# CompVis/unsupervised-part-segmentation

Measured on AMD Instinct MI355X. Metric: images/sec training (CUB 128x128, 10 parts), higher is better.
Workload: dtype bf16

## Files before the change

include/upsparts_hip.h:

```cpp
#ifndef UPSPARTS_HIP_H
#define UPSPARTS_HIP_H

#include <stddef.h>
#include <stdint.h>

#ifdef __cplusplus
extern "C" {
#endif

#define UPS_ABI_VERSION 6

enum { UPS_F32 = 0, UPS_BF16 = 1, UPS_F16 = 2 };
enum { UPS_ACT_NONE = 0, UPS_ACT_LRELU = 1, UPS_ACT_RELU = 2, UPS_ACT_ELU = 3 };
enum { UPS_OK = 0, UPS_E_ARG = -1, UPS_E_UNSUPPORTED = -2, UPS_E_LAUNCH = -3 };

int ups_abi_version(void);
void ups_struct_sizes(int64_t out[4]);
const char* ups_last_error(void);

typedef struct {
    int32_t dtype;
    int32_t n, hi, wi;
    int32_t ci;
    int32_t ldi;
// ... 137 lines not shown
int ups_act_mean_fwd(const void* x, void* y, int32_t dtype, int32_t n, int32_t hw, int32_t c, int32_t act, float slope, void* stream);
int ups_act_mean_bwd(const void* x, const void* gy, void* gx, int32_t dtype, int32_t n, int32_t hw, int32_t c, int32_t act, float slope, void* stream);
int ups_maxpool2_fwd(const void* x, void* y, int32_t dtype, int32_t n, int32_t h, int32_t w, int32_t c, void* stream);
int ups_maxpool2_fwd_f8(const void* x, void* y, int32_t n, int32_t h, int32_t w, int32_t c, void* y_f8, const float* scale,
                        float* amax, int32_t act, float slope, void* stream);
int ups_maxpool2_bwd(const void* x, const void* gy, void* gx, int32_t dtype, int32_t n, int32_t h, int32_t w, int32_t c, void* stream);
int ups_copy_channels(const void* src, int32_t lds, void* dst, int32_t ldd, int32_t dtype, int64_t rows, int32_t c, void* stream);
int ups_add_channels(const void* src, int32_t lds, void* dst, int32_t ldd, int32_t dtype, int64_t rows, int32_t c, void* stream);

int ups_vgg_preprocess_fwd(const void* x, int32_t x_is_f32, int32_t ldx, void* y, int32_t dtype, int64_t pixels, void* stream);
int ups_vgg_preprocess_bwd(const void* gy, void* gx, int32_t dtype, int32_t ldgx, int64_t pixels, void* stream);
int ups_l1_fwd(const void* a, const void* b, int32_t dtype, int64_t rows, int32_t c, int32_t ld, int32_t act,
               float* partial, int32_t nblocks, void* stream);
int ups_l1_bwd(const void* a, const void* b, void* gb, int32_t dtype, int64_t rows, int32_t c, int32_t ld, int32_t act,
               const float* scale_dev, float scale, void* stream);
int ups_sum_scale(const float* partial, int32_t n, float scale, float* out, int32_t accumulate, void* stream);

int ups_gram_plan(int32_t n, int64_t hw, int32_t c, int32_t dtype, int64_t* out);
int ups_gram_l1_fwd(const void* a, const void* b, int32_t dtype, int32_t n, int64_t hw, int32_t c, int32_t ld, int32_t act,
                    float* partial, void* sign, float* workspace, void* stream);
int ups_gram_l1_bwd(const void* b, const void* sign, void* gb, int32_t dtype, int32_t n, int64_t hw, int32_t c, int32_t ld,
                    int32_t act, const float* scale_dev, float scale, void* stream);

int ups_part_softmax_fwd(const float* mean, const float* eps, float* l, float* m, float* hard, int64_t* argmax,
                         uint32_t* hard_bits, int64_t pixels, int32_t P, void* stream);
int32_t ups_part_softmax_moments_tile(int32_t P);
size_t ups_part_softmax_moments_ints(int64_t pixels, int32_t P);
int ups_part_softmax_moments_fwd(const float* mean, const float* eps, float* l, float* m, float* hard, int64_t* argmax,
                                 uint32_t* hard_bits, int32_t n, int32_t h, int32_t w, int32_t P, float gamma, float* stats,
                                 int32_t* scratch, void* stream);
// ... 145 lines not shown
```

unsupervised-part-segmentation_amd/csrc/conv_aux.hip:

```cpp
#include "common.h"

namespace {

template <typename T>
__global__ void weight_prep_kernel(const float* __restrict__ src, int ntaps, int cin_v, int ci_log, int co,
                                   T* __restrict__ wf, int ci_pad, T* __restrict__ wd, int drows, int dk) {
    constexpr int BK = 64 / (int)sizeof(T);
    const int kcf = (ci_pad + BK - 1) / BK, kcd = (dk + BK - 1) / BK;
    const long long nf = wf ? (long long)ntaps * kcf * co * BK : 0;
    const long long nd = wd ? (long long)ntaps * kcd * drows * BK : 0;
    for (long long idx = (long long)blockIdx.x * blockDim.x + threadIdx.x; idx < nf + nd;
         idx += (long long)gridDim.x * blockDim.x) {
        if (idx < nf) {
            const int kk = (int)(idx % BK);
            long long t = idx / BK;
            const int c = (int)(t % co); t /= co;
            const int kc = (int)(t % kcf), tap = (int)(t / kcf);
            const int k = kc * BK + kk;
            const float v = k < ci_log ? src[((long long)tap * cin_v + k) * co + c] : 0.f;
            st_from_float<T>(wf + idx, v);
        } else {
            const long long j = idx - nf;
            const int kk = (int)(j % BK);
            long long t = j / BK;
// ... 23 lines not shown
        for (int s = 0; s < kw; ++s) {
            if (!((xm >> s) & 1)) continue;
            const float vx = V[((long long)(r * kw + s) * cin_v + ci_log) * co + c];
            const float vy = V[((long long)(r * kw + s) * cin_v + ci_log + 1) * co + c];
            const int dys = r == 0 ? dy[0] : (r == 1 ? dy[1] : dy[2]);
            const int dxs = s == 0 ? dx[0] : (s == 1 ? dx[1] : dx[2]);
            k0 = __fmaf_rn(__fmaf_rn(ax, (float)dxs, -1.f), vx, k0);
            k0 = __fmaf_rn(__fmaf_rn(ay, (float)dys, -1.f), vy, k0);
            kj = __fmaf_rn(sxj, vx, kj);
            ki = __fmaf_rn(syi, vy, ki);
        }
    }
}

template <typename T>
__device__ __forceinline__ void weight_prep_chunk(const ups_prep_item& it, long long blk0, float (*tile)[9]) {
    constexpr int BK = 64 / (int)sizeof(T);
    const long long idx = blk0 + threadIdx.x;
    const int kcf = (it.ci_pad + BK - 1) / BK, kcd = (it.dgrad_k + BK - 1) / BK;
    const long long nf = it.w_fwd ? (long long)it.ntaps * kcf * it.co * BK : 0;
    const long long nd = it.w_dgrad ? (long long)it.ntaps * kcd * it.dgrad_rows * BK : 0;
    const long long nc = it.ctab ? (long long)64 * it.co : 0;
    if (sizeof(T) == 2 && (it.co & 7) == 0 && blk0 + 256 <= nf && nf < (1ll << 31)) {
        unsigned t = (unsigned)(blk0 / BK);
        const int c0 = (int)(t % (unsigned)it.co); t /= (unsigned)it.co;
        const int kc = (int)(t % (unsigned)kcf), tap = (int)(t / (unsigned)kcf);
        const int rk = threadIdx.x >> 3, rc = threadIdx.x & 7;
        const int k = kc * BK + rk;
        __syncthreads();
        tile[rk][rc] = k < it.ci_log ? it.src[((long long)tap * it.cin_v + k) * it.co + c0 + rc] : 0.f;
        __syncthreads();
        st_from_float<T>((T*)it.w_fwd + idx, tile[threadIdx.x & 31][threadIdx.x >> 5]);
        return;
    }
    const bool small = nf + nd + nc < (1ll << 31);
    if (idx < nf) {
        int kk, c, kc, tap;
        if (small) {
            const unsigned u = (unsigned)idx;
            kk = (int)(u % BK);
            unsigned t = u / BK;
            c = (int)(t % (unsigned)it.co); t /= (unsigned)it.co;
            kc = (int)(t % (unsigned)kcf); tap = (int)(t / (unsigned)kcf);
        } else {
            kk = (int)(idx % BK);
            long long t = idx / BK;
            c = (int)(t % it.co); t /= it.co;
            kc = (int)(t % kcf); tap = (int)(t / kcf);
        }
// ... 19 lines not shown
    } else if (idx < nf + nd + nc) {
        const long long j = idx - nf - nd;
        const int c = (int)(j % it.co), cls = (int)(j / it.co);
        const int ym = cls >> 3, xm = cls & 7;
        float k0, kj, ki;
        coord_table_entry(it.src, it.kh, it.kw, it.cin_v, it.ci_log, it.co, c, ym, xm, it.dy, it.dx, it.in_sy, it.in_sx, it.ax, it.ay,
                          k0, kj, ki);
        it.ctab[((long long)cls * 3 + 0) * it.co + c] = k0;
        it.ctab[((long long)cls * 3 + 1) * it.co + c] = kj;
        it.ctab[((long long)cls * 3 + 2) * it.co + c] = ki;
    }
}

constexpr int PREP_CPB = 16;
constexpr int PREP_LDS_ITEMS = 1024;
template <typename T>
__global__ __launch_bounds__(256) void weight_prep_batch_kernel(const ups_prep_item* __restrict__ items,
                                                                const long long* __restrict__ prefix, int n_items, long long total_chunks) {
    __shared__ long long spre[PREP_LDS_ITEMS];
    __shared__ float tile[32][9];
    __shared__ float tile4[32][33];
    const bool in_lds = n_items <= PREP_LDS_ITEMS;
    if (in_lds) {
        for (int i = threadIdx.x; i < n_items; i += 256) spre[i] = prefix[i];
        __syncthreads();
    }
    const long long* pre = in_lds ? (const long long*)spre : prefix;
    int lo = -1;
    ups_prep_item it;
    for (int j = 0; j < PREP_CPB; ++j) {
        const long long b = (long long)blockIdx.x * PREP_CPB + j;
        if (b >= total_chunks) break;
        if (lo < 0 || (lo + 1 < n_items && pre[lo + 1] <= b)) {
            int l = 0, h = n_items - 1;
            while (l < h) {
                const int mid = (l + h + 1) >> 1;
                if (pre[mid] <= b) l = mid; else h = mid - 1;
            }
            lo = l;
            it = items[lo];
        }
        constexpr int BK = 64 / (int)sizeof(T);
        const long long c0i = b - pre[lo];
        if (sizeof(T) == 2 && (it.co & 31) == 0 && (c0i & 3) == 0 && j + 4 <= PREP_CPB && b + 4 <= total_chunks && it.w_fwd &&
            (((unsigned long long)it.src) & 15ull) == 0) {
            const int kcf = (it.ci_pad + BK - 1) / BK;
            const long long nf = (long long)it.ntaps * kcf * it.co * BK;
            if ((c0i + 4) * 256 <= nf && nf < (1ll << 31)) {
                unsigned t = (unsigned)(c0i * 256 / BK);
                const int c0 = (int)(t % (unsigned)it.co); t /= (unsigned)it.co;
                const int kc = (int)(t % (unsigned)kcf), tap = (int)(t / (unsigned)kcf);
                const int rk = threadIdx.x >> 3, rc = (threadIdx.x & 7) * 4;
                const int k = kc * BK + rk;
                __syncthreads();
                float4 v = make_float4(0.f, 0.f, 0.f, 0.f);
                if (k < it.ci_log) v = *(const float4*)(it.src + ((long long)tap * it.cin_v + k) * it.co + c0 + rc);
                tile4[rk][rc] = v.x; tile4[rk][rc + 1] = v.y; tile4[rk][rc + 2] = v.z; tile4[rk][rc + 3] = v.w;
                __syncthreads();
                T* dst = (T*)it.w_fwd + c0i * 256;
#pragma unroll
                for (int q = 0; q < 4; ++q) {
                    const int e = q * 256 + threadIdx.x;
                    st_from_float<T>(dst + e, tile4[e & 31][e >> 5]);
                }
                j += 3;
                continue;
            }
        }
        weight_prep_chunk<T>(it, c0i * 256, tile);
    }
}

struct Taps3 { int dy[3], dx[3]; };

__global__ void coord_table_kernel(const float* __restrict__ V, int kh, int kw, int ci_log, int co, Taps3 tp, int in_sy,
                                   int in_sx, float ax, float ay, float* __restrict__ tab) {
    const int cls = blockIdx.y;
    const int ym = cls >> 3, xm = cls & 7;
    const int c = blockIdx.x * blockDim.x + threadIdx.x;
    if (c >= co) return;
    float k0, kj, ki;
    coord_table_entry(V, kh, kw, ci_log + 2, ci_log, co, c, ym, xm, tp.dy, tp.dx, in_sy, in_sx, ax, ay, k0, kj, ki);
    tab[((long long)cls * 3 + 0) * co + c] = k0;
    tab[((long long)cls * 3 + 1) * co + c] = kj;
// ... 229 lines not shown
}

extern "C" int ups_weight_prep_d2s(const float* src, int32_t cin_v, int32_t ci_log, int32_t co, int32_t pad_y, int32_t pad_x,
                                   int32_t C, void* w, void* stream) {
    UPS_CHECK_ARG(src && w && ci_log >= 1 && cin_v >= ci_log && co >= 1 && C >= ci_log && C >= 8 && (C & (C - 1)) == 0);
    const int kc = (co + 31) / 32;
    const long long total = 9ll * kc * 4 * C * 4;
    hipLaunchKernelGGL(weight_prep_d2s_kernel, dim3((unsigned)((total + 255) / 256)), dim3(256), 0, (hipStream_t)stream, src, cin_v,
                       ci_log, co, pad_y, pad_x, C, kc, (uint4*)w, total);
    UPS_LAUNCH_CHECK();
    return UPS_OK;
}

extern "C" int64_t ups_prep_item_blocks(const ups_prep_item* item_host, int32_t dtype) {
    if (!item_host) return -1;
    return (prep_elems(*item_host, dtype == UPS_F32 ? 16 : 32) + 255) / 256;
}

extern "C" int ups_weight_prep_batch(const ups_prep_item* items, const int64_t* block_prefix, int32_t n_items,
                                     int64_t total_blocks, int32_t dtype, void* stream) {
    UPS_CHECK_ARG(items && block_prefix && n_items >= 1 && total_blocks >= 1 && total_blocks < 0x7fffffffLL);
    if (dtype == UPS_F32)
        hipLaunchKernelGGL(weight_prep_batch_kernel<float>, dim3((unsigned)ups_cdiv(total_blocks, PREP_CPB)), dim3(256), 0, (hipStream_t)stream,
                           items, (const long long*)block_prefix, n_items, (long long)total_blocks);
    else if (dtype == UPS_F16)
        hipLaunchKernelGGL(weight_prep_batch_kernel<f16>, dim3((unsigned)ups_cdiv(total_blocks, PREP_CPB)), dim3(256), 0, (hipStream_t)stream,
                           items, (const long long*)block_prefix, n_items, (long long)total_blocks);
    else
        hipLaunchKernelGGL(weight_prep_batch_kernel<bf16>, dim3((unsigned)ups_cdiv(total_blocks, PREP_CPB)), dim3(256), 0, (hipStream_t)stream,
                           items, (const long long*)block_prefix, n_items, (long long)total_blocks);
    UPS_LAUNCH_CHECK();
    return UPS_OK;
}

static Taps3 make_taps3(int kh, int kw, const int32_t* dy, const int32_t* dx) {
    Taps3 t;
    for (int i = 0; i < 3; ++i) { t.dy[i] = 0; t.dx[i] = 0; }
    for (int r = 0; r < kh; ++r) t.dy[r] = dy[r * kw];
    for (int s = 0; s < kw; ++s) t.dx[s] = dx[s];
    return t;
}

extern "C" int ups_coord_table(const float* V, int32_t kh, int32_t kw, int32_t ci_log, int32_t co, const int32_t* tap_dy,
                               const int32_t* tap_dx, int32_t in_sy, int32_t in_sx, float ax, float ay, float* tab,
// ... 62 lines not shown
```

unsupervised-part-segmentation_amd/csrc/pointwise.hip:

```cpp
#include "common.h"

namespace {

template <typename T> struct V16 {
    static constexpr int N = Chunk<T>::N;
    __device__ static inline void ld(const T* p, float* f) { uint4 u = *(const uint4*)p; Chunk<T>::unpack(u, f); }
    __device__ static inline void st(T* p, const float* f) { *(uint4*)p = Chunk<T>::pack(f); }
};

struct F8Emit {
    unsigned char* out;
    const float* scale; float* amax;
    int act, e5m2; float slope;
};
__device__ __forceinline__ void f8_emit_words(const F8Emit& q, float sc, float ns, long long elem, uint4 u, float& amax) {
    const unsigned w[4] = {u.x, u.y, u.z, u.w};
    ups_f32x2 f[4];
#pragma unroll
    for (int k = 0; k < 4; ++k) {
        f[k] = (ups_f32x2){__uint_as_float(w[k] << 16), __uint_as_float(w[k] & 0xffff0000u)};
        if (q.act != UPS_ACT_NONE) {
            const ups_f32x2 sx = f[k] * ns;
            f[k] = (ups_f32x2){ups_vmax(f[k][0], sx[0]), ups_vmax(f[k][1], sx[1])};
        }
// ... 388 lines not shown
#pragma unroll
    for (int e = 3; e < 8; ++e) st_from_float<T>(o + e, 0.f);
}
template <typename T>
__global__ void vgg_pre_bwd_kernel(const T* __restrict__ gy, T* __restrict__ gx, int ldgx, long long pixels) {
    const long long p = (long long)blockIdx.x * blockDim.x + threadIdx.x;
    if (p >= pixels) return;
    const T* g = gy + p * 8;
    T* o = gx + p * ldgx;
    st_from_float<T>(o + 0, 127.5f * ld_as_float<T>(g + 2));
    st_from_float<T>(o + 1, 127.5f * ld_as_float<T>(g + 1));
    st_from_float<T>(o + 2, 127.5f * ld_as_float<T>(g + 0));
    for (int e = 3; e < ldgx; ++e) st_from_float<T>(o + e, 0.f);
}

template <typename T>
__global__ __launch_bounds__(256) void l1_fwd_kernel(const T* __restrict__ a, const T* __restrict__ b, long long rows,
                                                     int c, int ld, int act, float* __restrict__ partial) {
    __shared__ float red[4];
    constexpr int E = V16<T>::N;
    const int cc = ld / E;
    const long long total = rows * cc;
    float s = 0.f;
    for (long long idx = (long long)blockIdx.x * blockDim.x + threadIdx.x; idx < total;
         idx += (long long)gridDim.x * blockDim.x) {
        const int k = (int)(idx % cc);
        float x[E], y[E];
        V16<T>::ld(a + idx * E, x);
        V16<T>::ld(b + idx * E, y);
#pragma unroll
        for (int e = 0; e < E; ++e)
            if (k * E + e < c) s += fabsf(ups_act(x[e], act, 0.f) - ups_act(y[e], act, 0.f));
    }
    s = block_sum_256(s, red);
    if (threadIdx.x == 0) partial[blockIdx.x] = s;
}
template <typename T>
__global__ void l1_bwd_kernel(const T* __restrict__ a, const T* __restrict__ b, T* __restrict__ gb, long long rows, int c,
                              int ld, int act, const float* __restrict__ scale_dev, float scale) {
    constexpr int E = V16<T>::N;
    const int cc = ld / E;
    const long long total = rows * cc;
    const float sc = scale * (scale_dev ? scale_dev[0] : 1.f);
    for (long long idx = (long long)blockIdx.x * blockDim.x + threadIdx.x; idx < total;
         idx += (long long)gridDim.x * blockDim.x) {
        const int k = (int)(idx % cc);
        float x[E], y[E], g[E];
        V16<T>::ld(a + idx * E, x);
        V16<T>::ld(b + idx * E, y);
#pragma unroll
        for (int e = 0; e < E; ++e) {
            const float d = ups_act(x[e], act, 0.f) - ups_act(y[e], act, 0.f);
            const float sg = d > 0.f ? 1.f : (d < 0.f ? -1.f : 0.f);
            g[e] = (k * E + e < c) ? -sc * sg * ups_dact(y[e], act, 0.f) : 0.f;
        }
        V16<T>::st(gb + idx * E, g);
    }
}

__global__ __launch_bounds__(256) void sum_scale_kernel(const float* __restrict__ partial, int n, float scale,
                                                        float* __restrict__ out, int accumulate) {
    __shared__ float red[4];
    float s = 0.f;
    for (int i = threadIdx.x; i < n; i += 256) s += partial[i];
    s = block_sum_256(s, red);
    if (threadIdx.x == 0) out[0] = (accumulate ? out[0] : 0.f) + scale * s;
}

template <typename TS, typename TD>
// ... 255 lines not shown
    else if (x_is_f32) hipLaunchKernelGGL((vgg_pre_fwd_kernel<bf16, float>), dim3(grid), dim3(256), 0, s, (const float*)x, ldx, (bf16*)y, (long long)pixels);
    else hipLaunchKernelGGL((vgg_pre_fwd_kernel<bf16, bf16>), dim3(grid), dim3(256), 0, s, (const bf16*)x, ldx, (bf16*)y, (long long)pixels);
    UPS_LAUNCH_CHECK();
    return UPS_OK;
}
extern "C" int ups_vgg_preprocess_bwd(const void* gy, void* gx, int32_t dtype, int32_t ldgx, int64_t pixels, void* stream) {
    UPS_CHECK_ARG(gy && gx && ldgx >= 3);
    UPS_CHECK_DTYPE_F32_BF16(dtype);
    hipStream_t s = (hipStream_t)stream;
    const int grid = ups_cdiv(pixels, 256);
    if (dtype == UPS_F32) hipLaunchKernelGGL(vgg_pre_bwd_kernel<float>, dim3(grid), dim3(256), 0, s, (const float*)gy, (float*)gx, ldgx, (long long)pixels);
    else hipLaunchKernelGGL(vgg_pre_bwd_kernel<bf16>, dim3(grid), dim3(256), 0, s, (const bf16*)gy, (bf16*)gx, ldgx, (long long)pixels);
    UPS_LAUNCH_CHECK();
    return UPS_OK;
}
extern "C" int ups_l1_fwd(const void* a, const void* b, int32_t dtype, int64_t rows, int32_t c, int32_t ld, int32_t act, float* partial, int32_t nblocks, void* stream) {
    UPS_CHECK_ARG(a && b && partial && ld % 8 == 0 && c <= ld && nblocks >= 1);
    UPS_CHECK_DTYPE_F32_BF16(dtype);
    hipStream_t s = (hipStream_t)stream;
    if (dtype == UPS_F32) hipLaunchKernelGGL(l1_fwd_kernel<float>, dim3(nblocks), dim3(256), 0, s, (const float*)a, (const float*)b, (long long)rows, c, ld, act, partial);
    else hipLaunchKernelGGL(l1_fwd_kernel<bf16>, dim3(nblocks), dim3(256), 0, s, (const bf16*)a, (const bf16*)b, (long long)rows, c, ld, act, partial);
    UPS_LAUNCH_CHECK();
    return UPS_OK;
}
extern "C" int ups_l1_bwd(const void* a, const void* b, void* gb, int32_t dtype, int64_t rows, int32_t c, int32_t ld, int32_t act, const float* scale_dev, float scale, void* stream) {
    UPS_CHECK_ARG(a && b && gb && ld % 8 == 0 && c <= ld);
    UPS_CHECK_DTYPE_F32_BF16(dtype);
    const long long work = (long long)rows * (ld / (dtype == UPS_F32 ? 4 : 8));
    hipStream_t s = (hipStream_t)stream;
    if (dtype == UPS_F32) hipLaunchKernelGGL(l1_bwd_kernel<float>, dim3(grid_for(work)), dim3(256), 0, s, (const float*)a, (const float*)b, (float*)gb, (long long)rows, c, ld, act, scale_dev, scale);
    else hipLaunchKernelGGL(l1_bwd_kernel<bf16>, dim3(grid_for(work)), dim3(256), 0, s, (const bf16*)a, (const bf16*)b, (bf16*)gb, (long long)rows, c, ld, act, scale_dev, scale);
    UPS_LAUNCH_CHECK();
    return UPS_OK;
}
extern "C" int ups_sum_scale(const float* partial, int32_t n, float scale, float* out, int32_t accumulate, void* stream) {
    UPS_CHECK_ARG(partial && out && n >= 1);
// ... 82 lines not shown
```

unsupervised-part-segmentation_amd/lib.py:

```python
import ctypes as C
import os

import torch

from . import switches as SW

_HERE = os.path.dirname(os.path.abspath(__file__))
LIB_PATH = SW.value("UPS_LIB") or os.path.join(_HERE, "csrc", "libupsparts_hip.so")

ABI_VERSION = 6
F32, BF16, F16 = 0, 1, 2
ACT_NONE, ACT_LRELU, ACT_RELU, ACT_ELU = 0, 1, 2, 3
ACT = {None: ACT_NONE, "leaky_relu": ACT_LRELU, "relu": ACT_RELU, "elu": ACT_ELU}


class UpsError(RuntimeError):
    pass


class ConvDesc(C.Structure):
    _fields_ = [("dtype", C.c_int32), ("n", C.c_int32), ("hi", C.c_int32), ("wi", C.c_int32), ("ci", C.c_int32),
                ("ldi", C.c_int32), ("ho", C.c_int32), ("wo", C.c_int32), ("co", C.c_int32), ("co_fill", C.c_int32),
                ("ldo", C.c_int32), ("out_h", C.c_int32), ("out_w", C.c_int32), ("out_sy", C.c_int32),
                ("out_sx", C.c_int32), ("out_oy", C.c_int32), ("out_ox", C.c_int32), ("in_sy", C.c_int32),
                ("in_sx", C.c_int32), ("ntaps", C.c_int32), ("kh", C.c_int32), ("kw", C.c_int32),
                ("tap_dy", C.c_int32 * 9), ("tap_dx", C.c_int32 * 9), ("tap_w", C.c_int32 * 9),
                ("act_in", C.c_int32), ("act_slope", C.c_float), ("out_f32", C.c_int32), ("dact_kind", C.c_int32),
# ... 78 lines not shown
    "ups_bilinear2x_fwd_f8": ([_P, _P, _I, _I, _I, _I, _P, _P, _P, _I, _F, _I, _P], C.c_int),
    "ups_bilinear2x_bwd_f8": ([_P, _P, _I, _I, _I, _I, _P, _P, _P, _I, _P], C.c_int),
    "ups_act_mean_fwd": ([_P, _P, _I, _I, _I, _I, _I, _F, _P], C.c_int),
    "ups_act_mean_bwd": ([_P, _P, _P, _I, _I, _I, _I, _I, _F, _P], C.c_int),
    "ups_elu_fwd": ([_P, _P, _I, C.c_int64, _P], C.c_int),
    "ups_elu_bwd": ([_P, _P, _P, _I, C.c_int64, _P], C.c_int),
    "ups_maxpool2_fwd": ([_P, _P, _I, _I, _I, _I, _I, _P], C.c_int),
    "ups_maxpool2_fwd_f8": ([_P, _P, _I, _I, _I, _I, _P, _P, _P, _I, _F, _P], C.c_int),
    "ups_maxpool2_bwd": ([_P, _P, _P, _I, _I, _I, _I, _I, _P], C.c_int),
    "ups_copy_channels": ([_P, _I, _P, _I, _I, _L, _I, _P], C.c_int),
    "ups_add_channels": ([_P, _I, _P, _I, _I, _L, _I, _P], C.c_int),
    "ups_vgg_preprocess_fwd": ([_P, _I, _I, _P, _I, _L, _P], C.c_int),
    "ups_vgg_preprocess_bwd": ([_P, _P, _I, _I, _L, _P], C.c_int),
    "ups_l1_fwd": ([_P, _P, _I, _L, _I, _I, _I, _P, _I, _P], C.c_int),
    "ups_l1_bwd": ([_P, _P, _P, _I, _L, _I, _I, _I, _P, _F, _P], C.c_int),
    "ups_sum_scale": ([_P, _I, _F, _P, _I, _P], C.c_int),
    "ups_gram_plan": ([_I, _L, _I, _I, C.POINTER(C.c_int64)], C.c_int),
    "ups_gram_l1_fwd": ([_P, _P, _I, _I, _L, _I, _I, _I, _P, _P, _P, _P], C.c_int),
    "ups_gram_l1_bwd": ([_P, _P, _P, _I, _I, _L, _I, _I, _I, _P, _F, _P], C.c_int),
    "ups_part_softmax_fwd": ([_P, _P, _P, _P, _P, _P, _P, _L, _I, _P], C.c_int),
    "ups_part_softmax_moments_tile": ([_I], _I),
    "ups_part_softmax_moments_ints": ([_L, _I], _Z),
    "ups_part_softmax_moments_fwd": ([_P, _P, _P, _P, _P, _P, _P, _I, _I, _I, _I, _F, _P, _P, _P], C.c_int),
    "ups_spatial_moments": ([_P, _I, _I, _I, _I, _F, _P, _I, _I, _P, _P], C.c_int),
    "ups_spatial_moments_kl": ([_P, _I, _I, _I, _I, _F, _P, _I, _I, _P, _P, _P], C.c_int),
    "ups_spatial_moments_floats": ([_I, _I], _Z),
    "ups_moments_to_px": ([_P, _I, _I, _I, _P, _P], C.c_int),
    "ups_draw_rect": ([_P, _I, _I, _I, _I, _I, _I, _P, _P], C.c_int),
    "ups_mask_parts_fwd": ([_P, _P, _P, _I, _I, _L, _I, _P], C.c_int),
    "ups_mask_parts_bwd": ([_P, _P, _P, _I, _I, _L, _I, _P], C.c_int),
# ... 123 lines not shown
```

unsupervised-part-segmentation_amd/ops.py:

```python
import ctypes as C
import os

import torch

from . import lib as L
from . import switches as SW


def round8(c):
    return (c + 7) // 8 * 8


def same_geometry(size, k, stride):
    out = -(-size // stride)
    pad_total = max((out - 1) * stride + k - size, 0)
    return out, pad_total // 2


class _Workspace(object):

    def __init__(self):
        self.bufs = {}

    def get(self, nbytes, device):
# ... 1205 lines not shown
        return y

    @staticmethod
    def backward(ctx, g):
        g = g.contiguous()
        assert ctx.in_dtype == g.dtype, "gradient flows back to an activation-dtype image"
        gx = torch.empty(ctx.in_shape, dtype=g.dtype, device=g.device)
        L.call("ups_vgg_preprocess_bwd", L.ptr(g), L.ptr(gx), L.dt(g), ctx.in_shape[-1],
               g.numel() // 8, L.stream())
        return gx, None


L1_BLOCKS = 1024


class L1MeanFn(torch.autograd.Function):

    @staticmethod
    def forward(ctx, a, b, c_log, act):
        a, b = a.contiguous(), b.contiguous()
        rows, ld = b.numel() // b.shape[-1], b.shape[-1]
        partial = torch.empty(L1_BLOCKS, dtype=torch.float32, device=b.device)
        out = torch.empty((), dtype=torch.float32, device=b.device)
        L.call("ups_l1_fwd", L.ptr(a), L.ptr(b), L.dt(b), rows, c_log, ld, act, L.ptr(partial), L1_BLOCKS, L.stream())
        L.call("ups_sum_scale", L.ptr(partial), L1_BLOCKS, 1.0 / (rows * c_log), L.ptr(out), 0, L.stream())
        ctx.save_for_backward(a, b)
        ctx.c_log, ctx.act = c_log, act
        return out

    @staticmethod
    def backward(ctx, g):
        a, b = ctx.saved_tensors
        rows, ld = b.numel() // b.shape[-1], b.shape[-1]
        gb = torch.empty_like(b)
        g = g.contiguous().float()
        L.call("ups_l1_bwd", L.ptr(a), L.ptr(b), L.ptr(gb), L.dt(b), rows, ctx.c_log, ld, ctx.act, L.ptr(g),
               1.0 / (rows * ctx.c_log), L.stream())
        return None, gb, None, None


GRAM_DIV = 4.0
_GRAM_PLANS = {}


def gram_plan(n, hw, c, dtype):
    key = (n, hw, c, dtype)
    if key not in _GRAM_PLANS:
        out = (C.c_int64 * 4)()
        L.check(L.load().ups_gram_plan(n, hw, c, dtype, out), "ups_gram_plan")
        _GRAM_PLANS[key] = tuple(int(v) for v in out)
    return _GRAM_PLANS[key]


class PerceptualTermFn(torch.autograd.Function):

    @staticmethod
    def forward(ctx, a, b, c_log, act, gram_w):
        a, b = a.contiguous(), b.contiguous()
        n, ld = b.shape[0], b.shape[-1]
        rows = b.numel() // ld
        hw = rows // n
        partial = torch.empty(L1_BLOCKS, dtype=torch.float32, device=b.device)
        out = torch.empty((), dtype=torch.float32, device=b.device)
        L.call("ups_l1_fwd", L.ptr(a), L.ptr(b), L.dt(b), rows, c_log, ld, act, L.ptr(partial), L1_BLOCKS, L.stream())
        L.call("ups_sum_scale", L.ptr(partial), L1_BLOCKS, 1.0 / (rows * c_log), L.ptr(out), 0, L.stream())
        _, npart, nws, nsign = gram_plan(n, hw, c_log, L.dt(b))
        gpart = torch.empty(npart, dtype=torch.float32, device=b.device)
        sign = torch.empty(nsign, dtype=torch.int8, device=b.device)
        ws = torch.empty(nws, dtype=torch.float32, device=b.device) if nws else None
        L.call("ups_gram_l1_fwd", L.ptr(a), L.ptr(b), L.dt(b), n, hw, c_log, ld, act, L.ptr(gpart), L.ptr(sign), L.ptr(ws),
               L.stream())
        norm = 1.0 / (GRAM_DIV * hw)
        L.call("ups_sum_scale", L.ptr(gpart), npart, gram_w * norm / (n * c_log * c_log), L.ptr(out), 1, L.stream())
        ctx.save_for_backward(a, b, sign)
        ctx.c_log, ctx.act, ctx.gram_w = c_log, act, gram_w
        return out

    @staticmethod
    def backward(ctx, g):
        a, b, sign = ctx.saved_tensors
        n, ld = b.shape[0], b.shape[-1]
        rows = b.numel() // ld
        hw, c_log = rows // n, ctx.c_log
        gb = torch.empty_like(b)
        g = g.contiguous().float()
        L.call("ups_l1_bwd", L.ptr(a), L.ptr(b), L.ptr(gb), L.dt(b), rows, c_log, ld, ctx.act, L.ptr(g),
               1.0 / (rows * c_log), L.stream())
        coef = 2.0 * ctx.gram_w / (n * c_log * c_log) / (GRAM_DIV * hw)
        L.call("ups_gram_l1_bwd", L.ptr(b), L.ptr(sign), L.ptr(gb), L.dt(b), n, hw, c_log, ld, ctx.act, L.ptr(g), coef, L.stream())
        return None, gb, None, None, None


class CriticHeadFn(torch.autograd.Function):

    @staticmethod
    def forward(ctx, h_pi, h_al, B, K):
        h_pi, h_al = h_pi.contiguous(), h_al.contiguous()
        ld = h_pi.shape[-1]
        assert h_pi.numel() == 2 * B * ld and h_al.shape == h_pi.shape
        logits = torch.empty(2 * B, dtype=torch.float32, device=h_pi.device)
        out = torch.empty(4, dtype=torch.float32, device=h_pi.device)
        L.call("ups_critic_head_fwd", L.ptr(h_pi), L.ptr(h_al), L.dt(h_pi), B, K, ld, L.ptr(logits), L.ptr(out), L.stream())
        ctx.save_for_backward(h_pi, h_al, logits)
        ctx.B, ctx.K = B, K
        loss, acc, mim = out[0], out[1], out[2]
# ... 635 lines not shown
```

Baseline: 2097.

## Save packed L1 sign codes for backward and retile bf16 weight prep

```diff
diff --git a/include/upsparts_hip.h b/include/upsparts_hip.h
--- a/include/upsparts_hip.h
+++ b/include/upsparts_hip.h
@@ -175,6 +175,9 @@
                float* partial, int32_t nblocks, void* stream);
 int ups_l1_bwd(const void* a, const void* b, void* gb, int32_t dtype, int64_t rows, int32_t c, int32_t ld, int32_t act,
                const float* scale_dev, float scale, void* stream);
+#define UPS_ACT_WITH_L1_CODES 0x100
+int ups_l1_bwd_codes(const void* codes, void* gb, int32_t dtype, int64_t rows, int32_t c, int32_t ld,
+                     const float* scale_dev, float scale, void* stream);
 int ups_sum_scale(const float* partial, int32_t n, float scale, float* out, int32_t accumulate, void* stream);
 
 int ups_gram_plan(int32_t n, int64_t hw, int32_t c, int32_t dtype, int64_t* out);
diff --git a/unsupervised-part-segmentation_amd/csrc/conv_aux.hip b/unsupervised-part-segmentation_amd/csrc/conv_aux.hip
--- a/unsupervised-part-segmentation_amd/csrc/conv_aux.hip
+++ b/unsupervised-part-segmentation_amd/csrc/conv_aux.hip
@@ -61,25 +61,13 @@
 }
 
 template <typename T>
-__device__ __forceinline__ void weight_prep_chunk(const ups_prep_item& it, long long blk0, float (*tile)[9]) {
+__device__ __forceinline__ void weight_prep_chunk(const ups_prep_item& it, long long blk0) {
     constexpr int BK = 64 / (int)sizeof(T);
     const long long idx = blk0 + threadIdx.x;
     const int kcf = (it.ci_pad + BK - 1) / BK, kcd = (it.dgrad_k + BK - 1) / BK;
     const long long nf = it.w_fwd ? (long long)it.ntaps * kcf * it.co * BK : 0;
     const long long nd = it.w_dgrad ? (long long)it.ntaps * kcd * it.dgrad_rows * BK : 0;
     const long long nc = it.ctab ? (long long)64 * it.co : 0;
-    if (sizeof(T) == 2 && (it.co & 7) == 0 && blk0 + 256 <= nf && nf < (1ll << 31)) {
-        unsigned t = (unsigned)(blk0 / BK);
-        const int c0 = (int)(t % (unsigned)it.co); t /= (unsigned)it.co;
-        const int kc = (int)(t % (unsigned)kcf), tap = (int)(t / (unsigned)kcf);
-        const int rk = threadIdx.x >> 3, rc = threadIdx.x & 7;
-        const int k = kc * BK + rk;
-        __syncthreads();
-        tile[rk][rc] = k < it.ci_log ? it.src[((long long)tap * it.cin_v + k) * it.co + c0 + rc] : 0.f;
-        __syncthreads();
-        st_from_float<T>((T*)it.w_fwd + idx, tile[threadIdx.x & 31][threadIdx.x >> 5]);
-        return;
-    }
     const bool small = nf + nd + nc < (1ll << 31);
     if (idx < nf) {
         int kk, c, kc, tap;
@@ -129,12 +117,19 @@
 
 constexpr int PREP_CPB = 16;
 constexpr int PREP_LDS_ITEMS = 1024;
+__device__ __forceinline__ int prep_find_item(const long long* pre, int n_items, long long b) {
+    int l = 0, h = n_items - 1;
+    while (l < h) {
+        const int mid = (l + h + 1) >> 1;
+        if (pre[mid] <= b) l = mid; else h = mid - 1;
+    }
+    return l;
+}
+
 template <typename T>
 __global__ __launch_bounds__(256) void weight_prep_batch_kernel(const ups_prep_item* __restrict__ items,
                                                                 const long long* __restrict__ prefix, int n_items, long long total_chunks) {
     __shared__ long long spre[PREP_LDS_ITEMS];
-    __shared__ float tile[32][9];
-    __shared__ float tile4[32][33];
     const bool in_lds = n_items <= PREP_LDS_ITEMS;
     if (in_lds) {
         for (int i = threadIdx.x; i < n_items; i += 256) spre[i] = prefix[i];
@@ -147,42 +142,130 @@
         const long long b = (long long)blockIdx.x * PREP_CPB + j;
         if (b >= total_chunks) break;
         if (lo < 0 || (lo + 1 < n_items && pre[lo + 1] <= b)) {
-            int l = 0, h = n_items - 1;
-            while (l < h) {
-                const int mid = (l + h + 1) >> 1;
-                if (pre[mid] <= b) l = mid; else h = mid - 1;
-            }
-            lo = l;
+            lo = prep_find_item(pre, n_items, b);
             it = items[lo];
         }
-        constexpr int BK = 64 / (int)sizeof(T);
-        const long long c0i = b - pre[lo];
-        if (sizeof(T) == 2 && (it.co & 31) == 0 && (c0i & 3) == 0 && j + 4 <= PREP_CPB && b + 4 <= total_chunks && it.w_fwd &&
-            (((unsigned long long)it.src) & 15ull) == 0) {
-            const int kcf = (it.ci_pad + BK - 1) / BK;
-            const long long nf = (long long)it.ntaps * kcf * it.co * BK;
-            if ((c0i + 4) * 256 <= nf && nf < (1ll << 31)) {
-                unsigned t = (unsigned)(c0i * 256 / BK);
-                const int c0 = (int)(t % (unsigned)it.co); t /= (unsigned)it.co;
-                const int kc = (int)(t % (unsigned)kcf), tap = (int)(t / (unsigned)kcf);
-                const int rk = threadIdx.x >> 3, rc = (threadIdx.x & 7) * 4;
-                const int k = kc * BK + rk;
-                __syncthreads();
+        weight_prep_chunk<T>(it, (b - pre[lo]) * 256);
+    }
+}
+
+constexpr int PREP_UPB = 8;
+struct PrepUnits { int kcf, cgf, kcd, rgd, kb, cb; long long nm, nc; };
+__host__ __device__ inline PrepUnits prep_units(const ups_prep_item& it) {
+    PrepUnits u;
+    u.kcf = it.w_fwd ? (it.ci_pad + 31) / 32 : 0; u.cgf = it.w_fwd ? (it.co + 31) / 32 : 0;
+    u.kcd = it.w_dgrad ? (it.dgrad_k + 31) / 32 : 0; u.rgd = it.w_dgrad ? (it.dgrad_rows + 31) / 32 : 0;
+    u.kb = u.kcf > u.rgd ? u.kcf : u.rgd;
+    u.cb = u.cgf > u.kcd ? u.cgf : u.kcd;
+    u.nm = (long long)it.ntaps * u.kb * u.cb;
+    u.nc = it.ctab ? ((long long)64 * it.co + 127) / 128 : 0;
+    return u;
+}
+
+template <typename T>
+__device__ __forceinline__ void prep_store8(T* dst, const float* f, bool vec) {
+    if (vec) *(uint4*)dst = Chunk<T>::pack(f);
+    else {
+#pragma unroll
+        for (int e = 0; e < 8; ++e) st_from_float<T>(dst + e, f[e]);
+    }
+}
+
+template <typename T>
+__global__ __launch_bounds__(256) void weight_prep_units_kernel(const ups_prep_item* __restrict__ items,
+                                                                const long long* __restrict__ prefix, int n_items, long long total_units) {
+    static_assert(sizeof(T) == 2, "16-bit layouts: 32 elements per 64-byte row");
+    __shared__ long long spre[PREP_LDS_ITEMS];
+    __shared__ float tile[2][32][33];
+    const bool in_lds = n_items <= PREP_LDS_ITEMS;
+    if (in_lds) {
+        for (int i = threadIdx.x; i < n_items; i += 256) spre[i] = prefix[i];
+        __syncthreads();
+    }
+    const long long* pre = in_lds ? (const long long*)spre : prefix;
+    const int h = threadIdx.x >> 7, t = threadIdx.x & 127;
+    int lo = -1;
+    ups_prep_item it;
+    PrepUnits pu;
+    bool vsrc = false;
+    for (int j = 0; j < PREP_UPB / 2; ++j) {
+        const long long u0 = (long long)blockIdx.x * PREP_UPB + 2 * j;
+        if (u0 >= total_units) break;
+        const long long u = u0 + h;
+        int kind = 0;
+        int tap = 0, kb = 0, cb = 0;
+        unsigned ui = 0;
+        if (u < total_units) {
+            if (lo < 0 || (lo + 1 < n_items && pre[lo + 1] <= u)) {
+                lo = prep_find_item(pre, n_items, u);
+                it = items[lo];
+                pu = prep_units(it);
+                vsrc = (it.co & 3) == 0 && (((unsigned long long)it.src) & 15ull) == 0;
+            }
+            ui = (unsigned)(u - pre[lo]);
+            if (ui < pu.nm) {
+                kind = 1;
+                const unsigned q = ui / (unsigned)pu.cb;
+                cb = (int)(ui - q * (unsigned)pu.cb);
+                tap = (int)(q / (unsigned)pu.kb); kb = (int)(q - (unsigned)tap * (unsigned)pu.kb);
+            } else if (ui < pu.nm + pu.nc) {
+                kind = 2;
+            }
+        }
+        __syncthreads();
+        if (kind == 1) {
+#pragma unroll
+            for (int q = 0; q < 2; ++q) {
+                const int p = t + 128 * q, rk = p >> 3, rc = (p & 7) * 4;
+                const int k = kb * 32 + rk, c = cb * 32 + rc;
                 float4 v = make_float4(0.f, 0.f, 0.f, 0.f);
-                if (k < it.ci_log) v = *(const float4*)(it.src + ((long long)tap * it.cin_v + k) * it.co + c0 + rc);
-                tile4[rk][rc] = v.x; tile4[rk][rc + 1] = v.y; tile4[rk][rc + 2] = v.z; tile4[rk][rc + 3] = v.w;
-                __syncthreads();
-                T* dst = (T*)it.w_fwd + c0i * 256;
-#pragma unroll
-                for (int q = 0; q < 4; ++q) {
-                    const int e = q * 256 + threadIdx.x;
-                    st_from_float<T>(dst + e, tile4[e & 31][e >> 5]);
+                if (k < it.ci_log) {
+                    const float* s = it.src + ((long long)tap * it.cin_v + k) * it.co + c;
+                    if (vsrc) { if (c < it.co) v = *(const float4*)s; }
+                    else {
+                        if (c < it.co) v.x = s[0];
+                        if (c + 1 < it.co) v.y = s[1];
+                        if (c + 2 < it.co) v.z = s[2];
+                        if (c + 3 < it.co) v.w = s[3];
+                    }
                 }
-                j += 3;
-                continue;
-            }
-        }
-        weight_prep_chunk<T>(it, c0i * 256, tile);
+                tile[h][rk][rc] = v.x; tile[h][rk][rc + 1] = v.y; tile[h][rk][rc + 2] = v.z; tile[h][rk][rc + 3] = v.w;
+            }
+        }
+        __syncthreads();
+        if (kind == 1) {
+            const int rl = t >> 2, kq = (t & 3) * 8;
+            float f[8];
+            if (kb < pu.kcf && cb < pu.cgf) {
+                const int c = cb * 32 + rl;
+                if (c < it.co) {
+#pragma unroll
+                    for (int e = 0; e < 8; ++e) f[e] = tile[h][kq + e][rl];
+                    T* dst = (T*)it.w_fwd + (((long long)tap * pu.kcf + kb) * it.co + c) * 32 + kq;
+                    prep_store8<T>(dst, f, (((unsigned long long)it.w_fwd) & 15ull) == 0);
+                }
+            }
+            if (kb < pu.rgd && cb < pu.kcd) {
+                const int r = kb * 32 + rl;
+                if (r < it.dgrad_rows) {
+#pragma unroll
+                    for (int e = 0; e < 8; ++e) f[e] = tile[h][rl][kq + e];
+                    T* dst = (T*)it.w_dgrad + (((long long)tap * pu.kcd + cb) * it.dgrad_rows + r) * 32 + kq;
+                    prep_store8<T>(dst, f, (((unsigned long long)it.w_dgrad) & 15ull) == 0);
+                }
+            }
+        } else if (kind == 2) {
+            const long long e = (long long)(ui - (unsigned)pu.nm) * 128 + t;
+            if (e < (long long)64 * it.co) {
+                const int c = (int)(e % it.co), cls = (int)(e / it.co);
+                float k0, kj, ki;
+                coord_table_entry(it.src, it.kh, it.kw, it.cin_v, it.ci_log, it.co, c, cls >> 3, cls & 7, it.dy, it.dx, it.in_sy, it.in_sx,
+                                  it.ax, it.ay, k0, kj, ki);
+                it.ctab[((long long)cls * 3 + 0) * it.co + c] = k0;
+                it.ctab[((long long)cls * 3 + 1) * it.co + c] = kj;
+                it.ctab[((long long)cls * 3 + 2) * it.co + c] = ki;
+            }
+        }
     }
 }
 
@@ -442,7 +525,9 @@
 
 extern "C" int64_t ups_prep_item_blocks(const ups_prep_item* item_host, int32_t dtype) {
     if (!item_host) return -1;
-    return (prep_elems(*item_host, dtype == UPS_F32 ? 16 : 32) + 255) / 256;
+    if (dtype == UPS_F32) return (prep_elems(*item_host, 16) + 255) / 256;
+    const PrepUnits u = prep_units(*item_host);
+    return u.nm + u.nc;
 }
 
 extern "C" int ups_weight_prep_batch(const ups_prep_item* items, const int64_t* block_prefix, int32_t n_items,
@@ -452,10 +537,10 @@
         hipLaunchKernelGGL(weight_prep_batch_kernel<float>, dim3((unsigned)ups_cdiv(total_blocks, PREP_CPB)), dim3(256), 0, (hipStream_t)stream,
                            items, (const long long*)block_prefix, n_items, (long long)total_blocks);
     else if (dtype == UPS_F16)
-        hipLaunchKernelGGL(weight_prep_batch_kernel<f16>, dim3((unsigned)ups_cdiv(total_blocks, PREP_CPB)), dim3(256), 0, (hipStream_t)stream,
+        hipLaunchKernelGGL(weight_prep_units_kernel<f16>, dim3((unsigned)ups_cdiv(total_blocks, PREP_UPB)), dim3(256), 0, (hipStream_t)stream,
                            items, (const long long*)block_prefix, n_items, (long long)total_blocks);
     else
-        hipLaunchKernelGGL(weight_prep_batch_kernel<bf16>, dim3((unsigned)ups_cdiv(total_blocks, PREP_CPB)), dim3(256), 0, (hipStream_t)stream,
+        hipLaunchKernelGGL(weight_prep_units_kernel<bf16>, dim3((unsigned)ups_cdiv(total_blocks, PREP_UPB)), dim3(256), 0, (hipStream_t)stream,
                            items, (const long long*)block_prefix, n_items, (long long)total_blocks);
     UPS_LAUNCH_CHECK();
     return UPS_OK;
diff --git a/unsupervised-part-segmentation_amd/csrc/pointwise.hip b/unsupervised-part-segmentation_amd/csrc/pointwise.hip
--- a/unsupervised-part-segmentation_amd/csrc/pointwise.hip
+++ b/unsupervised-part-segmentation_amd/csrc/pointwise.hip
@@ -426,9 +426,13 @@
     for (int e = 3; e < ldgx; ++e) st_from_float<T>(o + e, 0.f);
 }
 
-template <typename T>
+template <typename T> struct L1Code;
+template <> struct L1Code<bf16> { typedef unsigned short type; };
+template <> struct L1Code<float> { typedef unsigned char type; };
+template <typename T, bool CODES>
 __global__ __launch_bounds__(256) void l1_fwd_kernel(const T* __restrict__ a, const T* __restrict__ b, long long rows,
-                                                     int c, int ld, int act, float* __restrict__ partial) {
+                                                     int c, int ld, int act, float* __restrict__ partial,
+                                                     typename L1Code<T>::type* __restrict__ codes) {
     __shared__ float red[4];
     constexpr int E = V16<T>::N;
     const int cc = ld / E;
@@ -440,9 +444,18 @@
         float x[E], y[E];
         V16<T>::ld(a + idx * E, x);
         V16<T>::ld(b + idx * E, y);
-#pragma unroll
-        for (int e = 0; e < E; ++e)
-            if (k * E + e < c) s += fabsf(ups_act(x[e], act, 0.f) - ups_act(y[e], act, 0.f));
+        unsigned code = 0;
+#pragma unroll
+        for (int e = 0; e < E; ++e) {
+            const float d = ups_act(x[e], act, 0.f) - ups_act(y[e], act, 0.f);
+            if (k * E + e < c) s += fabsf(d);
+            if (CODES) {
+                const unsigned neg = d < 0.f ? 1u : 0u;
+                const unsigned on = (fabsf(d) > 0.f && (act != UPS_ACT_RELU || y[e] > 0.f)) ? 2u : 0u;
+                code |= (neg | on) << (2 * e);
+            }
+        }
+        if (CODES) codes[idx] = (typename L1Code<T>::type)code;
     }
     s = block_sum_256(s, red);
     if (threadIdx.x == 0) partial[blockIdx.x] = s;
@@ -465,6 +478,27 @@
             const float d = ups_act(x[e], act, 0.f) - ups_act(y[e], act, 0.f);
             const float sg = d > 0.f ? 1.f : (d < 0.f ? -1.f : 0.f);
             g[e] = (k * E + e < c) ? -sc * sg * ups_dact(y[e], act, 0.f) : 0.f;
+        }
+        V16<T>::st(gb + idx * E, g);
+    }
+}
+template <typename T>
+__global__ void l1_bwd_codes_kernel(const typename L1Code<T>::type* __restrict__ codes, T* __restrict__ gb, long long rows, int c,
+                                    int ld, const float* __restrict__ scale_dev, float scale) {
+    constexpr int E = V16<T>::N;
+    const int cc = ld / E;
+    const long long total = rows * cc;
+    const float sc = scale * (scale_dev ? scale_dev[0] : 1.f);
+    for (long long idx = (long long)blockIdx.x * blockDim.x + threadIdx.x; idx < total;
+         idx += (long long)gridDim.x * blockDim.x) {
+        const int k = (int)(idx % cc);
+        const unsigned code = codes[idx];
+        float g[E];
+#pragma unroll
+        for (int e = 0; e < E; ++e) {
+            const float sg = ((code >> (2 * e)) & 1u) ? -1.f : 1.f;
+            const float da = ((code >> (2 * e)) & 2u) ? 1.f : 0.f;
+            g[e] = (k * E + e < c) ? -sc * sg * da : 0.f;
         }
         V16<T>::st(gb + idx * E, g);
     }
@@ -750,12 +784,37 @@
     UPS_LAUNCH_CHECK();
     return UPS_OK;
 }
+static int l1_fwd_launch(const void* a, const void* b, int32_t dtype, int64_t rows, int32_t c, int32_t ld, int32_t act, float* partial,
+                         int32_t nblocks, void* codes, void* stream) {
+    hipStream_t s = (hipStream_t)stream;
+    if (dtype == UPS_F32) {
+        if (codes) hipLaunchKernelGGL((l1_fwd_kernel<float, true>), dim3(nblocks), dim3(256), 0, s, (const float*)a, (const float*)b, (long long)rows, c, ld, act, partial, (unsigned char*)codes);
+        else hipLaunchKernelGGL((l1_fwd_kernel<float, false>), dim3(nblocks), dim3(256), 0, s, (const float*)a, (const float*)b, (long long)rows, c, ld, act, partial, (unsigned char*)nullptr);
+    } else {
+        if (codes) hipLaunchKernelGGL((l1_fwd_kernel<bf16, true>), dim3(nblocks), dim3(256), 0, s, (const bf16*)a, (const bf16*)b, (long long)rows, c, ld, act, partial, (unsigned short*)codes);
+        else hipLaunchKernelGGL((l1_fwd_kernel<bf16, false>), dim3(nblocks), dim3(256), 0, s, (const bf16*)a, (const bf16*)b, (long long)rows, c, ld, act, partial, (unsigned short*)nullptr);
+    }
+    UPS_LAUNCH_CHECK();
+    return UPS_OK;
+}
 extern "C" int ups_l1_fwd(const void* a, const void* b, int32_t dtype, int64_t rows, int32_t c, int32_t ld, int32_t act, float* partial, int32_t nblocks, void* stream) {
     UPS_CHECK_ARG(a && b && partial && ld % 8 == 0 && c <= ld && nblocks >= 1);
     UPS_CHECK_DTYPE_F32_BF16(dtype);
-    hipStream_t s = (hipStream_t)stream;
-    if (dtype == UPS_F32) hipLaunchKernelGGL(l1_fwd_kernel<float>, dim3(nblocks), dim3(256), 0, s, (const float*)a, (const float*)b, (long long)rows, c, ld, act, partial);
-    else hipLaunchKernelGGL(l1_fwd_kernel<bf16>, dim3(nblocks), dim3(256), 0, s, (const bf16*)a, (const bf16*)b, (long long)rows, c, ld, act, partial);
+    void* codes = nullptr;
+    if (act & UPS_ACT_WITH_L1_CODES) {
+        act &= ~UPS_ACT_WITH_L1_CODES;
+        UPS_CHECK_ARG(act == UPS_ACT_NONE || act == UPS_ACT_RELU);
+        codes = partial + nblocks;
+    }
+    return l1_fwd_launch(a, b, dtype, rows, c, ld, act, partial, nblocks, codes, stream);
+}
+extern "C" int ups_l1_bwd_codes(const void* codes, void* gb, int32_t dtype, int64_t rows, int32_t c, int32_t ld, const float* scale_dev, float scale, void* stream) {
+    UPS_CHECK_ARG(codes && gb && ld % 8 == 0 && c <= ld);
+    UPS_CHECK_DTYPE_F32_BF16(dtype);
+    const long long work = (long long)rows * (ld / (dtype == UPS_F32 ? 4 : 8));
+    hipStream_t s = (hipStream_t)stream;
+    if (dtype == UPS_F32) hipLaunchKernelGGL(l1_bwd_codes_kernel<float>, dim3(grid_for(work)), dim3(256), 0, s, (const unsigned char*)codes, (float*)gb, (long long)rows, c, ld, scale_dev, scale);
+    else hipLaunchKernelGGL(l1_bwd_codes_kernel<bf16>, dim3(grid_for(work)), dim3(256), 0, s, (const unsigned short*)codes, (bf16*)gb, (long long)rows, c, ld, scale_dev, scale);
     UPS_LAUNCH_CHECK();
     return UPS_OK;
 }
diff --git a/unsupervised-part-segmentation_amd/lib.py b/unsupervised-part-segmentation_amd/lib.py
--- a/unsupervised-part-segmentation_amd/lib.py
+++ b/unsupervised-part-segmentation_amd/lib.py
@@ -11,6 +11,7 @@
 ABI_VERSION = 6
 F32, BF16, F16 = 0, 1, 2
 ACT_NONE, ACT_LRELU, ACT_RELU, ACT_ELU = 0, 1, 2, 3
+ACT_WITH_L1_CODES = 0x100
 ACT = {None: ACT_NONE, "leaky_relu": ACT_LRELU, "relu": ACT_RELU, "elu": ACT_ELU}
 
 
@@ -119,6 +120,7 @@
     "ups_vgg_preprocess_bwd": ([_P, _P, _I, _I, _L, _P], C.c_int),
     "ups_l1_fwd": ([_P, _P, _I, _L, _I, _I, _I, _P, _I, _P], C.c_int),
     "ups_l1_bwd": ([_P, _P, _P, _I, _L, _I, _I, _I, _P, _F, _P], C.c_int),
+    "ups_l1_bwd_codes": ([_P, _P, _I, _L, _I, _I, _P, _F, _P], C.c_int),
     "ups_sum_scale": ([_P, _I, _F, _P, _I, _P], C.c_int),
     "ups_gram_plan": ([_I, _L, _I, _I, C.POINTER(C.c_int64)], C.c_int),
     "ups_gram_l1_fwd": ([_P, _P, _I, _I, _L, _I, _I, _I, _P, _P, _P, _P], C.c_int),
diff --git a/unsupervised-part-segmentation_amd/ops.py b/unsupervised-part-segmentation_amd/ops.py
--- a/unsupervised-part-segmentation_amd/ops.py
+++ b/unsupervised-part-segmentation_amd/ops.py
@@ -1243,29 +1243,55 @@
 L1_BLOCKS = 1024
 
 
+def _l1_forward(ctx, a, b, c_log, act, taped):
+    rows, ld = b.numel() // b.shape[-1], b.shape[-1]
+    if taped and ctx.needs_input_grad[1] and act in (L.ACT_NONE, L.ACT_RELU):
+        buf = torch.empty(L1_BLOCKS * 4 + rows * ld // 4, dtype=torch.uint8, device=b.device)
+        partial, codes = buf[:L1_BLOCKS * 4].view(torch.float32), buf[L1_BLOCKS * 4:]
+        act |= L.ACT_WITH_L1_CODES
+    else:
+        partial, codes = torch.empty(L1_BLOCKS, dtype=torch.float32, device=b.device), None
+    L.call("ups_l1_fwd", L.ptr(a), L.ptr(b), L.dt(b), rows, c_log, ld, act, L.ptr(partial), L1_BLOCKS, L.stream())
+    return partial, codes
+
+
 class L1MeanFn(torch.autograd.Function):
 
-    @staticmethod
-    def forward(ctx, a, b, c_log, act):
+    @classmethod
+    def apply(cls, a, b, c_log, act):
+        return super(L1MeanFn, cls).apply(a, b, c_log, act, torch.is_grad_enabled())
+
+    @staticmethod
+    def forward(ctx, a, b, c_log, act, taped=False):
         a, b = a.contiguous(), b.contiguous()
         rows, ld = b.numel() // b.shape[-1], b.shape[-1]
-        partial = torch.empty(L1_BLOCKS, dtype=torch.float32, device=b.device)
         out = torch.empty((), dtype=torch.float32, device=b.device)
-        L.call("ups_l1_fwd", L.ptr(a), L.ptr(b), L.dt(b), rows, c_log, ld, act, L.ptr(partial), L1_BLOCKS, L.stream())
+        partial, codes = _l1_forward(ctx, a, b, c_log, act, taped)
         L.call("ups_sum_scale", L.ptr(partial), L1_BLOCKS, 1.0 / (rows * c_log), L.ptr(out), 0, L.stream())
-        ctx.save_for_backward(a, b)
+        if codes is not None:
+            ctx.save_for_backward(codes)
+            ctx.b_shape, ctx.b_dtype = b.shape, b.dtype
+        else:
+            ctx.save_for_backward(a, b)
         ctx.c_log, ctx.act = c_log, act
         return out
 
     @staticmethod
     def backward(ctx, g):
+        g = g.contiguous().float()
+        if len(ctx.saved_tensors) == 1:
+            codes, = ctx.saved_tensors
+            gb = torch.empty(ctx.b_shape, dtype=ctx.b_dtype, device=codes.device)
+            rows, ld = gb.numel() // gb.shape[-1], gb.shape[-1]
+            L.call("ups_l1_bwd_codes", L.ptr(codes), L.ptr(gb), L.dt(gb), rows, ctx.c_log, ld, L.ptr(g), 1.0 / (rows * ctx.c_log),
+                   L.stream())
+            return None, gb, None, None, None
         a, b = ctx.saved_tensors
         rows, ld = b.numel() // b.shape[-1], b.shape[-1]
         gb = torch.empty_like(b)
-        g = g.contiguous().float()
         L.call("ups_l1_bwd", L.ptr(a), L.ptr(b), L.ptr(gb), L.dt(b), rows, ctx.c_log, ld, ctx.act, L.ptr(g),
                1.0 / (rows * ctx.c_log), L.stream())
-        return None, gb, None, None
+        return None, gb, None, None, None
 
 
 GRAM_DIV = 4.0
@@ -1283,15 +1309,18 @@
 
 class PerceptualTermFn(torch.autograd.Function):
 
-    @staticmethod
-    def forward(ctx, a, b, c_log, act, gram_w):
+    @classmethod
+    def apply(cls, a, b, c_log, act, gram_w):
+        return super(PerceptualTermFn, cls).apply(a, b, c_log, act, gram_w, torch.is_grad_enabled())
+
+    @staticmethod
+    def forward(ctx, a, b, c_log, act, gram_w, taped=False):
         a, b = a.contiguous(), b.contiguous()
         n, ld = b.shape[0], b.shape[-1]
         rows = b.numel() // ld
         hw = rows // n
-        partial = torch.empty(L1_BLOCKS, dtype=torch.float32, device=b.device)
         out = torch.empty((), dtype=torch.float32, device=b.device)
-        L.call("ups_l1_fwd", L.ptr(a), L.ptr(b), L.dt(b), rows, c_log, ld, act, L.ptr(partial), L1_BLOCKS, L.stream())
+        partial, codes = _l1_forward(ctx, a, b, c_log, act, taped)
         L.call("ups_sum_scale", L.ptr(partial), L1_BLOCKS, 1.0 / (rows * c_log), L.ptr(out), 0, L.stream())
         _, npart, nws, nsign = gram_plan(n, hw, c_log, L.dt(b))
         gpart = torch.empty(npart, dtype=torch.float32, device=b.device)
@@ -1301,23 +1330,33 @@
                L.stream())
         norm = 1.0 / (GRAM_DIV * hw)
         L.call("ups_sum_scale", L.ptr(gpart), npart, gram_w * norm / (n * c_log * c_log), L.ptr(out), 1, L.stream())
-        ctx.save_for_backward(a, b, sign)
+        if codes is not None:
+            ctx.save_for_backward(b, sign, codes)
+        else:
+            ctx.save_for_backward(a, b, sign)
+        ctx.l1_codes = codes is not None
         ctx.c_log, ctx.act, ctx.gram_w = c_log, act, gram_w
         return out
 
     @staticmethod
     def backward(ctx, g):
-        a, b, sign = ctx.saved_tensors
+        if ctx.l1_codes:
+            b, sign, codes = ctx.saved_tensors
+        else:
+            a, b, sign = ctx.saved_tensors
         n, ld = b.shape[0], b.shape[-1]
         rows = b.numel() // ld
         hw, c_log = rows // n, ctx.c_log
         gb = torch.empty_like(b)
         g = g.contiguous().float()
-        L.call("ups_l1_bwd", L.ptr(a), L.ptr(b), L.ptr(gb), L.dt(b), rows, c_log, ld, ctx.act, L.ptr(g),
-               1.0 / (rows * c_log), L.stream())
+        if ctx.l1_codes:
+            L.call("ups_l1_bwd_codes", L.ptr(codes), L.ptr(gb), L.dt(b), rows, c_log, ld, L.ptr(g), 1.0 / (rows * c_log), L.stream())
+        else:
+            L.call("ups_l1_bwd", L.ptr(a), L.ptr(b), L.ptr(gb), L.dt(b), rows, c_log, ld, ctx.act, L.ptr(g),
+                   1.0 / (rows * c_log), L.stream())
         coef = 2.0 * ctx.gram_w / (n * c_log * c_log) / (GRAM_DIV * hw)
         L.call("ups_gram_l1_bwd", L.ptr(b), L.ptr(sign), L.ptr(gb), L.dt(b), n, hw, c_log, ld, ctx.act, L.ptr(g), coef, L.stream())
-        return None, gb, None, None, None
+        return None, gb, None, None, None, None
 
 
 class CriticHeadFn(torch.autograd.Function):
```

Result: no change. 2113 (median of 6 runs) (+0.8%).
